# microsoft/SpeechT5

Measured on AMD Instinct MI355X. Metric: audio-sec/s fwd+bwd SpeechT5-Base, higher is better.
Workload: dtype bf16

## Files before the change

### include/speecht5_hip.h

```cpp
#ifndef SPEECHT5_HIP_H
#define SPEECHT5_HIP_H
#include <stdint.h>
#ifdef __cplusplus
extern "C" {
#endif

#define ST5_F32 0
#define ST5_BF16 1

#define ST5_ACT_NONE 0
#define ST5_ACT_GELU 1
#define ST5_ACT_RELU 2
#define ST5_ACT_TANH 3
#define ST5_ACT_LRELU_01 4
#define ST5_ACT_LRELU_001 5

#define ST5_GEMM_A_KSTRIDED 1
#define ST5_GEMM_B_KSTRIDED 2
#define ST5_GEMM_OUT_F32 4
#define ST5_GEMM_DACT 8
#define ST5_GEMM_DEFERRABLE 16

typedef struct st5_operand {
  const void* ptr;
// ... 124 lines not shown
                               const uint8_t* kpm, int32_t B, int32_t H, int32_t T, int32_t S, int32_t head_dim, int32_t nb,
                               int32_t maxrel, int32_t causal, int32_t lds, float scale, float dropout_p, uint64_t seed,
                               const float* gate, int32_t dkv_live, int dtype, void* stream, void* stream2);

int st5_conv0_gn_gelu_fwd(const float* wav, const float* w, const float* gamma, const float* beta, void* out,
                          float* stats, void* ws, int32_t B, int32_t S, int32_t C, int32_t k, int32_t stride,
                          float eps, int dtype, void* stream);
int st5_conv0_gn_gelu_bwd(const float* wav, const float* w, const float* gamma, const float* beta,
                          const float* stats, const void* dY, float* dw, float* dgamma, float* dbeta, void* ws,
                          int32_t B, int32_t S, int32_t C, int32_t k, int32_t stride, float gscale, int dtype,
                          void* stream);
int32_t st5_conv0_mom_count(int32_t k);
int st5_conv0_gn_gelu_fwd_m(const float* wav, const float* w, const float* gamma, const float* beta, void* out, float* stats, double* mom,
                            void* ws, int32_t B, int32_t S, int32_t C, int32_t k, int32_t stride, float eps, int dtype, void* stream);
int st5_conv0_gn_gelu_bwd_m(const float* wav, const float* w, const float* gamma, const float* beta, const float* stats, const double* mom,
                            const void* dY, float* dw, float* dgamma, float* dbeta, void* ws, int32_t B, int32_t S, int32_t C, int32_t k,
                            int32_t stride, float gscale, int dtype, void* stream);
int st5_conv0_gn_gelu_fwd_rows(const float* wav, const int32_t* lens, const float* w, const float* gamma, const float* beta, void* out,
                               float* stats, void* ws, int32_t B, int32_t S, int32_t C, int32_t k, int32_t stride, float eps, int dtype,
                               void* stream);
int st5_conv0_set_mfma(int on);
int st5_conv0_set_fold(int on);
int st5_conv0_set_gelu_table(int on);
int64_t st5_conv0_ws_bytes(int32_t B, int32_t S, int32_t C, int32_t k, int32_t stride);

int st5_cast_from_f32(const float* src, void* dst, int64_t rows, int64_t cols, int32_t transpose, int dtype,
                      void* stream);
int st5_cast_to_f32(const void* src, float* dst, int64_t n, int dtype, void* stream);
int st5_colsum_ws(const void* x, float* out, void* ws, int64_t rows, int32_t cols, int64_t ld, float scale,
                  int32_t accumulate, int dtype, void* stream);
int st5_colsum_ws_gate(const void* x, float* out, void* ws, int64_t rows, int32_t cols, int64_t ld, float scale, int32_t accumulate,
                       const float* gate, int dtype, void* stream);
int64_t st5_colsum_ws_bytes(int64_t rows, int32_t cols);
int st5_sumsq(const void* x, float* out, int64_t n, float scale, int32_t accumulate, int dtype, void* stream);
int st5_axpby(const void* x, void* y, int64_t n, float a, float b, int dtype, void* stream);
int st5_select(const float* keep_dev, const void* a, const void* b, void* y, int64_t nbytes, void* stream);
int st5_select_bwd(const float* keep_dev, const void* g, void* ga, void* gb, int64_t nbytes, void* stream);
int st5_skip_grad(const float* keep_dev, const void* g, void* dx, int64_t nbytes, void* stream);
int st5_act_fwd(const void* x, void* y, int64_t n, int32_t act, int dtype, void* stream);
int st5_act_bwd(const void* dy, const void* x, void* dx, int64_t n, int32_t act, int dtype, void* stream);
int st5_channel_affine(const void* x, const float* a, const float* b, void* y, int64_t rows, int32_t cols, int32_t act,
                       int dtype, void* stream);
int st5_dropout(const void* x, void* y, int64_t n, float p, uint64_t seed, int dtype, void* stream);
int st5_masked_fill_rows(void* x, const uint8_t* mask, const float* v, int64_t rows, int32_t cols, int dtype,
                         void* stream);
int st5_masked_fill_rows_bwd(void* dx, const uint8_t* mask, float* dv, int64_t rows, int32_t cols, int dtype,
                             void* stream);
int st5_add_table_rows(const void* x, const float* table, const int32_t* idx, void* y, int64_t rows, int32_t cols,
                       float scale, int dtype, void* stream);
int st5_add_table_rows_dev(const void* x, const float* table, const int32_t* idx, void* y, int64_t rows, int32_t cols,
                           const float* scale_dev, int dtype, void* stream);
int st5_embed_rows(const float* table, const int32_t* tok, const float* pos, const int32_t* pidx, void* y,
                   int64_t rows, int32_t cols, float emb_scale, float pos_scale, int dtype, void* stream);
int st5_embed_rows_bwd(const void* dy, const int32_t* tok, float* dtable, int64_t rows, int32_t cols, float scale,
                       int dtype, void* stream);
int st5_embed_rows_bwd_det(const void* dy, const int32_t* tok, float* dtable, int64_t rows, int32_t cols, int32_t vocab, float scale,
                           int dtype, void* stream);
int st5_embed_rows_bwd_det_w(const void* dy, const int32_t* tok, float* dtable, int64_t rows, int32_t cols, int32_t vocab, float scale,
                             const float* row_w, int32_t rw_div, int32_t rw_mod, int dtype, void* stream);
int st5_gather3(const float* src, void* dst, int32_t A, int32_t B, int32_t C, int64_t sa, int64_t sb, int64_t sc, int64_t off,
                int32_t accumulate, int dtype, void* stream);
int st5_zero_time_edges(void* x, int32_t B, int32_t Tp, int32_t C, int32_t head, int32_t tail_start, int dtype, void* stream);
int st5_unfold_rows(const float* wav, void* out, int32_t B, int32_t S, int32_t k, int32_t stride, int32_t kpad, int dtype,
                    void* stream);
int st5_pad_time(const void* src, void* dst, int32_t B, int32_t T, int32_t C, int32_t pad_l, int32_t pad_r,
                 int dtype, void* stream);
// ... 154 lines not shown
```

### speecht5_amd/csrc/flash_attn2.hip

```cpp
#include "common.h"
#include "../../include/speecht5_hip.h"

#ifndef FA2_ABL
#define FA2_ABL 0
#endif
#ifdef FA2_DMA_NOP
#define FA2_AFTER_DMA(p) asm volatile("s_nop 7\n\ts_nop 7" ::"v"(p) : "memory")
#else
#define FA2_AFTER_DMA(p)
#endif
namespace fa2 {

constexpr int HD = 64;
constexpr int KT = 64;
constexpr int TILE_B = KT * HD * 2;
constexpr int QP_PAD = 8;
constexpr int WIN = 104;
constexpr int WCH = 13;
constexpr int SCR_B = 7168;
constexpr float LOG2E = 1.4426950408889634f;
constexpr float LN2 = 0.6931471805599453f;
constexpr unsigned int PAIR_MUL = 0x9E3779B1u;

typedef __attribute__((address_space(3))) void* lds_ptr_t;
// ... 506 lines not shown
  block_coords(xb_, bh);
  const int b = bh / a.H, h = bh % a.H;
  const int qblk = xb_ * 128;
  const int qw0 = qblk + wave * 32;
  const int qi = qw0 + ql;
  const int qc = qi < a.T ? qi : a.T - 1;
  const bool qvalid = qi < a.T;

  bf16x8 qf[4], dof[4];
#pragma unroll
  for (int ks = 0; ks < 4; ++ks) {
    qf[ks] = *reinterpret_cast<const bf16x8*>(a.q + ((long long)b * a.T + qc) * a.q_ld + h * HD + ks * 16 + hi * 8);
    dof[ks] = *reinterpret_cast<const bf16x8*>(a.dout + ((long long)b * a.T + qc) * a.do_ld + h * HD + ks * 16 + hi * 8);
  }
  const float lse2 = a.lse[(long long)bh * a.T + qc] * LOG2E;
  float dsum;
  if (a.dvec_in_dq) {
    float part = 0.f;
#pragma unroll
    for (int ks = 0; ks < 4; ++ks) {
      const bf16x8 of = *reinterpret_cast<const bf16x8*>(a.o + ((long long)b * a.T + qc) * a.o_ld + h * HD + ks * 16 + hi * 8);
#pragma unroll
      for (int e = 0; e < 8; ++e) part = fmaf((float)dof[ks][e], (float)of[e], part);
    }
    dsum = part + __shfl_xor(part, 32, 64);
    if (qvalid && hi == 0) a.dvec[(long long)bh * a.T + qi] = dsum;
  } else {
    dsum = a.dvec[(long long)bh * a.T + qc];
  }

  if (BIAS && a.dvec_in_dq) {
    const int nrows = a.T - qblk < 128 ? a.T - qblk : 128;
    uint4* zp = reinterpret_cast<uint4*>(a.dqp + ((long long)bh * a.T + qblk) * a.nb);
    const int n16 = nrows * (a.nb >> 3);
    for (int i = tid; i < n16; i += 256) zp[i] = make_uint4(0u, 0u, 0u, 0u);
    asm volatile("s_waitcnt vmcnt(0)" ::: "memory");
    __builtin_amdgcn_s_barrier();
  }
  int nkeys = a.S;
  if (a.causal) {
    const int qmax = (qblk + 127 < a.T ? qblk + 127 : a.T - 1) + (a.S - a.T);
    nkeys = qmax + 1 < a.S ? qmax + 1 : a.S;
  }
  const int ntiles = (nkeys + KT - 1) / KT;
  const bf16_t* kbase = a.k + (long long)b * a.S * a.k_ld + h * HD;
  const bf16_t* vbase = a.v + (long long)b * a.S * a.v_ld + h * HD;
  TileStager ts;
  ts.init(wave, lane);
  const int nbp = a.nb + 2 * QP_PAD;
  const bf16_t* qpb = BIAS ? a.qp + (long long)bh * a.T * nbp : nullptr;
  WinStager wsg;
  if (BIAS) wsg.init(lane, qw0, a.T, nbp);
  float blo = 0.f, bhi = 0.f;
  if (BIAS) {
    blo = (float)qpb[(long long)qc * nbp];
    bhi = (float)qpb[(long long)qc * nbp + QP_PAD + a.nb];
  }
  TrAddr tra;
  tra.init(lane);
  int koff[2][2];
#pragma unroll
  for (int dt = 0; dt < 2; ++dt) {
    koff[dt][0] = tra.off(4 * hi, dt);
    koff[dt][1] = tra.off(8 + 4 * hi, dt);
  }
  const uint8_t* mrow = a.kpm ? a.kpm + (long long)b * a.S : nullptr;
  unsigned int raw_next = kpm_raw(mrow, lane, a.S);

  ts.issue(kbase, a.k_ld, 0, a.S, kbuf, wave);
  ts.issue(vbase, a.v_ld, 0, a.S, vbuf, wave);
// ... 683 lines not shown
```

### speecht5_amd/csrc/norm.hip

```cpp
#include "common.h"
#include "../../include/speecht5_hip.h"

namespace {

constexpr int MAXCH = 8;

template <typename T, int NCH>
__device__ __forceinline__ void load_row(const T* row, int cols, int lane, bool vec, float (&v)[NCH][8]) {
#pragma unroll
  for (int i = 0; i < NCH; ++i) {
    const int c = i * 512 + lane * 8;
    if (c < cols) {
      if (vec) load8f<T>(row + c, v[i]);
      else {
#pragma unroll
        for (int e = 0; e < 8; ++e) v[i][e] = (c + e < cols) ? Elem<T>::to_f(row[c + e]) : 0.f;
      }
    } else {
#pragma unroll
      for (int e = 0; e < 8; ++e) v[i][e] = 0.f;
    }
  }
}
template <typename T, int NCH>
// ... 467 lines not shown
        }
        const float mu = mean[r], rs = rstd[r];
#pragma unroll
        for (int e = 0; e < 8; ++e) acc[e] += b[e] * (a[e] - mu) * rs;
      } else {
#pragma unroll
        for (int e = 0; e < 8; ++e) acc[e] += a[e];
      }
    }
  }
#pragma unroll
  for (int e = 0; e < 8; ++e) red[ty][tx * 8 + e] = acc[e];
  __syncthreads();
  const int c = threadIdx.x;
  if (blockIdx.x * 256 + c < cols) {
    float s = 0.f;
#pragma unroll
    for (int j = 0; j < 8; ++j) s += red[j][c];
    part[(long long)blockIdx.y * cols + blockIdx.x * 256 + c] = s;
  }
}
__global__ void colreduce_final_kernel(const float* __restrict__ part, float* __restrict__ out, int nsplit, int cols,
                                       float scale, int accumulate, const float* __restrict__ gate = nullptr) {
  const int c = blockIdx.x * blockDim.x + threadIdx.x;
  if (c >= cols) return;
  if (st5_gate_dropped(gate)) {
    if (!accumulate) out[c] = 0.f;
    return;
  }
  float s = 0.f;
  for (int j = 0; j < nsplit; ++j) s += part[(long long)j * cols + c];
  s *= scale;
  out[c] = accumulate ? out[c] + s : s;
}

int nsplit_for(long long rows) {
  long long n = (rows + 63) / 64;
  if (n < 1) n = 1;
  if (n > 64) n = 64;
  return (int)n;
}

template <typename T, int MODE>
int colreduce(const void* x, const void* dy, const float* mean, const float* rstd, float* out, float* ws,
              long long rows, int cols, long long ld, float scale, int accumulate, hipStream_t s, const float* gate = nullptr) {
  const int ns = nsplit_for(rows);
  dim3 grid((cols + 255) / 256, ns);
  hipLaunchKernelGGL((colreduce_kernel<T, MODE>), grid, dim3(256), 0, s, (const T*)x, (const T*)dy, mean, rstd, ws,
                     rows, cols, ld, gate);
  hipLaunchKernelGGL(colreduce_final_kernel, dim3((cols + 255) / 256), dim3(256), 0, s, ws, out, ns, cols, scale,
                     accumulate, gate);
  HIP_CHECK_LAUNCH();
  return ST5_OK;
}

}

static int layernorm_fwd(const void* x, const float* gamma, const float* beta, void* y, float* mean,
                         float* rstd, int64_t rows, int32_t cols, float eps, int dtype, void* stream, const float* keep, const void* skip,
                         const float* gate = nullptr) {
  if (!x || !y || !gamma || !beta || rows < 0 || cols <= 0 || cols > MAXCH * 512) return ST5_ERR_ARG;
  if (keep && (!skip || cols % 4 != 0 || cols > 2048)) return ST5_ERR_ARG;
  if (gate && ((skip && !keep) || cols % 4 != 0 || cols > 2048)) return ST5_ERR_ARG;
  if (rows == 0) return ST5_OK;
  hipStream_t s = (hipStream_t)stream;
  dim3 grid((unsigned)((rows + 3) / 4));
// ... 226 lines not shown
#undef g_ln_arena_bytes
#undef g_ln_arena_used
extern "C" int st5_layernorm_defer(int enabled, void* stream) {
  (void)stream;
  if (!enabled && g_ln_defer) {
    for (int i = 0; i < g_nlnstates; ++i) { const int rc = ln_flush_state(&g_lnstates[i]); if (rc) return rc; }
  }
  g_ln_defer = enabled != 0;
  return ST5_OK;
}
extern "C" int st5_layernorm_flush(void* stream) { return ln_flush(reinterpret_cast<hipStream_t>(stream)); }
extern "C" int st5_layernorm_set_max_blocks(int n) { if (n < 1 || n > 4096) return ST5_ERR_ARG; g_ln_max_blocks = n; return ST5_OK; }

extern "C" int st5_colsum_ws(const void* x, float* out, void* ws, int64_t rows, int32_t cols, int64_t ld, float scale,
                             int32_t accumulate, int dtype, void* stream) {
  if (!x || !out || !ws || rows < 0 || cols <= 0) return ST5_ERR_ARG;
  hipStream_t s = (hipStream_t)stream;
  if (dtype == ST5_BF16)
    return colreduce<bf16_t, 0>(x, nullptr, nullptr, nullptr, out, (float*)ws, rows, cols, ld, scale, accumulate, s);
  if (dtype == ST5_F32)
    return colreduce<float, 0>(x, nullptr, nullptr, nullptr, out, (float*)ws, rows, cols, ld, scale, accumulate, s);
  return ST5_ERR_ARG;
}
extern "C" int st5_colsum_ws_gate(const void* x, float* out, void* ws, int64_t rows, int32_t cols, int64_t ld, float scale,
                                  int32_t accumulate, const float* gate, int dtype, void* stream) {
  if (!x || !out || !ws || rows < 0 || cols <= 0) return ST5_ERR_ARG;
  hipStream_t s = (hipStream_t)stream;
  if (dtype == ST5_BF16)
    return colreduce<bf16_t, 0>(x, nullptr, nullptr, nullptr, out, (float*)ws, rows, cols, ld, scale, accumulate, s, gate);
  if (dtype == ST5_F32)
    return colreduce<float, 0>(x, nullptr, nullptr, nullptr, out, (float*)ws, rows, cols, ld, scale, accumulate, s, gate);
  return ST5_ERR_ARG;
}
extern "C" int64_t st5_colsum_ws_bytes(int64_t rows, int32_t cols) {
  return (int64_t)nsplit_for(rows) * cols * sizeof(float);
}
```

### speecht5_amd/functional.py

```python
import math
from types import SimpleNamespace

import os
import threading

import torch

from . import hip
from .hip import ACT_GELU, ACT_NONE, ACT_RELU, ACT_TANH

_S = SimpleNamespace(dtype=torch.float32, seed=0x5EED, counter=0, grad_hook=None, boundary_hook=None, side=None, side_raw=0,
                     side_keep=[], side_gens=[], side_n=0, attn_side=None, attn_side_raw=None, slots=None, force_static=False)


def set_compute_dtype(dtype):
    assert dtype in (torch.float32, torch.bfloat16)
    _S.dtype = dtype


def compute_dtype():
    return _S.dtype


def manual_seed(seed):
# ... 1520 lines not shown
    hip.gemm(hip.operand(dS, lds, **zP), hip.operand(kt, kld, off=koff, zs0=S * kld, zs1=hd),
             hip.operand(dqt, dqld, off=dqoff, zs0=T * dqld, zs1=hd), T, hd, S, _dt(dtype), batch=BH, zdiv=H,
             flags=hip.B_KSTRIDED, alpha=alpha)
    if pe is not None:
        hip.gemm(hip.operand(dqp, nb, zs0=H * T * nb, zs1=T * nb), hip.operand(pe, hd),
                 hip.operand(dqt, dqld, off=dqoff, zs0=T * dqld, zs1=hd), T, hd, nb, _dt(dtype), batch=BH, zdiv=H,
                 flags=hip.B_KSTRIDED, alpha=alpha, beta=1.0)
    hip.gemm(hip.operand(dS, lds, **zP), hip.operand(qt, qld, off=qoff, zs0=T * qld, zs1=hd),
             hip.operand(dkt, dkld, off=dkoff, zs0=S * dkld, zs1=hd), S, hd, T, _dt(dtype), batch=BH, zdiv=H,
             flags=hip.A_KSTRIDED | hip.B_KSTRIDED, alpha=alpha)
    if pe is not None and want_dpe:
        part = torch.empty(BH, nb, hd, dtype=torch.float32, device=dev)
        hip.gemm(hip.operand(dqp, nb, zs0=H * T * nb, zs1=T * nb),
                 hip.operand(qt, qld, off=qoff, zs0=T * qld, zs1=hd),
                 hip.operand(part, hd, zs0=H * nb * hd, zs1=nb * hd), nb, hd, T, _dt(dtype), batch=BH, zdiv=H,
                 flags=hip.A_KSTRIDED | hip.B_KSTRIDED | hip.OUT_F32, alpha=alpha)
        g = torch.zeros(nb, hd, dtype=torch.float32, device=dev)
        L = hip.lib()
        ws = hip.workspace(L.st5_colsum_ws_bytes(BH, nb * hd), dev)
        hip.check(L.st5_colsum_ws(part.data_ptr(), g.data_ptr(), ws.data_ptr(), BH, nb * hd, nb * hd, 1.0, 1, hip.F32,
                                  hip.stream()), "st5_colsum_ws")
        return g
    return None



_FLASH = SimpleNamespace(enabled=True)


def set_flash_attention(enabled):
    _FLASH.enabled = bool(enabled)


def _can_flash(dtype, hd, want_probs):
    return _FLASH.enabled and dtype == torch.bfloat16 and hd == 64 and not want_probs


def _eptr(t3):
    t, _ld, off = t3
    return t.data_ptr() + off * t.element_size()


_LOG2E = 1.4426950408889634


def _flash_fwd(q, k, v, B, H, T, S, hd, pe, maxrel, kpm, causal, p_drop, seed, save_qp=False):
    dev = q[0].device
    d = H * hd
    ctx = _gout(torch.empty(B * T, d, dtype=torch.bfloat16, device=dev))
    lse = _gout(torch.empty(B * H, T, dtype=torch.float32, device=dev))
    nb = pe.shape[0] if pe is not None else 0
    qp = _gout(torch.empty(B * H, T, hip.lib().st5_flash_attn_qp_row(nb), dtype=torch.bfloat16, device=dev)) if pe is not None else None
    if hip.gate():
        hip.check(hip.lib().st5_flash_attn_fwd_qp_gate(_eptr(q), q[1], _eptr(k), k[1], _eptr(v), v[1], ctx.data_ptr(), d, lse.data_ptr(),
                                                       hip.ptr(pe), hip.ptr(kpm), B, H, T, S, hd, nb, maxrel, 1 if causal else 0, _ceil8(S),
                                                       hd ** -0.5, p_drop, seed, hip.ptr(qp), hip.gate(), hip.BF16, hip.stream()),
                  "st5_flash_attn_fwd_qp_gate")
        return ctx, lse, (qp if save_qp else None)
    hip.check(hip.lib().st5_flash_attn_fwd_qp(_eptr(q), q[1], _eptr(k), k[1], _eptr(v), v[1], ctx.data_ptr(), d, lse.data_ptr(),
                                              hip.ptr(pe), hip.ptr(kpm), B, H, T, S, hd, nb, maxrel, 1 if causal else 0, _ceil8(S),
                                              hd ** -0.5, p_drop, seed, hip.ptr(qp), hip.BF16, hip.stream()), "st5_flash_attn_fwd_qp")
    return ctx, lse, (qp if save_qp else None)


def set_attention_stream(stream):
    _S.attn_side = stream
# ... 16 lines not shown
    lg = hip.gate()
    dev = dctx.device
    dtype = torch.bfloat16
    d = H * hd
    BH = B * H
    alpha = hd ** -0.5
    dvec = _gout(torch.empty(BH * T, dtype=torch.float32, device=dev))
    dqp = None
    nb = 0
    qt, qld, qoff = q
    if pe is not None:
        nb = pe.shape[0]
        assert qp is not None or not lg, "a gated layer keeps the forward's relative-position table (st5_flash_attn_qp_table carries no gate)"
        if qp is None:
            qp = torch.empty(BH, T, hip.lib().st5_flash_attn_qp_row(nb), dtype=dtype, device=dev)
            hip.check(hip.lib().st5_flash_attn_qp_table(_eptr(q), q[1], pe.data_ptr(), qp.data_ptr(), B, H, T, nb, alpha, hip.BF16,
                                                        hip.stream()), "st5_flash_attn_qp_table")
        dqp = _gout(torch.empty(BH, T, nb, dtype=dtype, device=dev))
    if lg:
        hip.check(hip.lib().st5_flash_attn_bwd_2s_gate(_eptr(q), q[1], _eptr(k), k[1], _eptr(v), v[1], ctx.data_ptr(), d, dctx.data_ptr(), d,
                                                       _eptr(dq), dq[1], _eptr(dk), dk[1], _eptr(dv), dv[1], lse.data_ptr(), dvec.data_ptr(),
                                                       hip.ptr(pe), hip.ptr(qp), hip.ptr(dqp), hip.ptr(kpm), B, H, T, S, hd, nb, maxrel,
                                                       1 if causal else 0, _ceil8(S), alpha, p_drop, seed, lg, 1 if dkv_live else 0, hip.BF16,
                                                       hip.stream(), _attn_side_raw()), "st5_flash_attn_bwd_2s_gate")
    else:
        hip.check(hip.lib().st5_flash_attn_bwd_2s(_eptr(q), q[1], _eptr(k), k[1], _eptr(v), v[1], ctx.data_ptr(), d, dctx.data_ptr(), d,
                                                  _eptr(dq), dq[1], _eptr(dk), dk[1], _eptr(dv), dv[1], lse.data_ptr(), dvec.data_ptr(),
                                                  hip.ptr(pe), hip.ptr(qp), hip.ptr(dqp), hip.ptr(kpm), B, H, T, S, hd, nb, maxrel,
                                                  1 if causal else 0, _ceil8(S), alpha, p_drop, seed, hip.BF16, hip.stream(),
                                                  _attn_side_raw()), "st5_flash_attn_bwd_2s")
    if pe is None:
        return None
    dqt, dqld, dqoff = dq
    if pe_t is not None:
        hip.gemm(hip.operand(dqp, nb, zs0=H * T * nb, zs1=T * nb), hip.operand(pe_t, nb),
                 hip.operand(dqt, dqld, off=dqoff, zs0=T * dqld, zs1=hd), T, hd, nb, hip.BF16, batch=BH, zdiv=H, alpha=alpha, beta=1.0)
    else:
        hip.gemm(hip.operand(dqp, nb, zs0=H * T * nb, zs1=T * nb), hip.operand(pe, hd),
                 hip.operand(dqt, dqld, off=dqoff, zs0=T * dqld, zs1=hd), T, hd, nb, hip.BF16, batch=BH, zdiv=H,
                 flags=hip.B_KSTRIDED, alpha=alpha, beta=1.0)
    if not want_dpe:
        return None
    part = _gout(torch.empty(BH, nb, hd, dtype=torch.float32, device=dev))
    hip.gemm(hip.operand(dqp, nb, zs0=H * T * nb, zs1=T * nb), hip.operand(qt, qld, off=qoff, zs0=T * qld, zs1=hd),
             hip.operand(part, hd, zs0=H * nb * hd, zs1=nb * hd), nb, hd, T, hip.BF16, batch=BH, zdiv=H,
             flags=hip.A_KSTRIDED | hip.B_KSTRIDED | hip.OUT_F32, alpha=alpha)
    g = _gout(torch.empty(nb, hd, dtype=torch.float32, device=dev))
    L = hip.lib()
    ws = hip.workspace(L.st5_colsum_ws_bytes(BH, nb * hd), dev)
    if lg:
        hip.check(L.st5_colsum_ws_gate(part.data_ptr(), g.data_ptr(), ws.data_ptr(), BH, nb * hd, nb * hd, 1.0, 0, lg, hip.F32, hip.stream()),
                  "st5_colsum_ws_gate")
        return g
    hip.check(L.st5_colsum_ws(part.data_ptr(), g.data_ptr(), ws.data_ptr(), BH, nb * hd, nb * hd, 1.0, 0, hip.F32, hip.stream()),
              "st5_colsum_ws")
    return g


class SelfAttentionFunction(torch.autograd.Function):

    @staticmethod
    @_lg_fwd
    def forward(ctx_, qkv, pe, kpm, cfg):
        B, H, T, hd, maxrel, causal, p_drop = cfg[:7]
        d = H * hd
        seed = next_seed() if p_drop > 0 else 0
        assert _LG.keep is None or _can_flash(qkv.dtype, hd, False), "gated layer without the fused attention kernels"
        if _can_flash(qkv.dtype, hd, False):
            ctx, lse, qp = _flash_fwd((qkv, 3 * d, 0), (qkv, 3 * d, d), (qkv, 3 * d, 2 * d), B, H, T, T, hd, pe, maxrel, kpm, causal,
                                      p_drop, seed, save_qp=any(ctx_.needs_input_grad))
            ctx_.save_for_backward(qkv, ctx, lse, pe, kpm, qp)
            ctx_.meta = (cfg, seed, True)
            return ctx
        ctx, probs, pdrop = _attn_fwd((qkv, 3 * d, 0), (qkv, 3 * d, d), (qkv, 3 * d, 2 * d), B, H, T, T, hd, pe, maxrel,
                                      kpm, causal, p_drop, seed)
        ctx_.save_for_backward(qkv, probs, pdrop, pe)
        ctx_.meta = (cfg, seed, False)
        return ctx

    @staticmethod
    @_lg_bwd
    def backward(ctx_, dctx):
        cfg, seed, flash = ctx_.meta
        B, H, T, hd, maxrel, causal, p_drop = cfg[:7]
        pe_t = cfg[7] if len(cfg) > 7 else None
        d = H * hd
        if flash:
            qkv, ctx, lse, pe, kpm, qp = ctx_.saved_tensors
            dqkv = _gout(torch.empty_like(qkv))
            dpe = _flash_bwd(dctx.contiguous(), ctx, lse, (qkv, 3 * d, 0), (qkv, 3 * d, d), (qkv, 3 * d, 2 * d), (dqkv, 3 * d, 0),
                             (dqkv, 3 * d, d), (dqkv, 3 * d, 2 * d), B, H, T, T, hd, pe, pe is not None and ctx_.needs_input_grad[1],
                             maxrel, kpm, causal, p_drop, seed, qp=qp, pe_t=pe_t)
            if dpe is not None and pe.dtype != torch.float32:
                dpe = to_compute(dpe)
            return dqkv, dpe, None, None
        qkv, probs, pdrop, pe = ctx_.saved_tensors
        dqkv = torch.empty_like(qkv)
        dpe = _attn_bwd(dctx.contiguous(), (qkv, 3 * d, 0), (qkv, 3 * d, d), (qkv, 3 * d, 2 * d), (dqkv, 3 * d, 0),
                        (dqkv, 3 * d, d), (dqkv, 3 * d, 2 * d), probs, pdrop, None, B, H, T, T, hd, pe,
                        pe is not None and ctx_.needs_input_grad[1], maxrel, p_drop, seed)
        if dpe is not None and pe.dtype != torch.float32:
            dpe = to_compute(dpe)
        return dqkv, dpe, None, None


class KVShare:

    def __init__(self, n_layers, width, may_skip_layers):
        self.n_layers, self.width, self.may_skip = n_layers, width, may_skip_layers
        self.first = None
        self.grad = None

    def grad_buffer(self, like):
        if self.grad is None:
            self.grad = (torch.zeros_like if self.may_skip else torch.empty_like)(like)
        return self.grad


class CrossAttentionFunction(torch.autograd.Function):

    @staticmethod
    @_lg_fwd
    def forward(ctx_, q, kv, kpm, cfg):
        B, H, T, S, hd, p_drop, want_probs = cfg[:7]
        d = H * hd
        kld, koff, share = cfg[7:10] if len(cfg) > 7 else (2 * d, 0, None)
# ... 1398 lines not shown
```

### speecht5_amd/hip.py

```python
import ctypes
import os
from ctypes import POINTER, Structure, byref, c_char_p, c_float, c_int, c_int32, c_int64, c_uint64, c_void_p

import torch

F32, BF16 = 0, 1
ACT_NONE, ACT_GELU, ACT_RELU, ACT_TANH, ACT_LRELU_01, ACT_LRELU_001 = 0, 1, 2, 3, 4, 5
A_KSTRIDED, B_KSTRIDED, OUT_F32, DACT = 1, 2, 4, 8
DEFERRABLE = 16

_LIB_PATH = os.environ.get("ST5_HIP_LIB") or os.path.join(os.path.dirname(os.path.abspath(__file__)), "libspeecht5_hip.so")


class HipLibraryMissing(RuntimeError):
    pass


class HipKernelError(RuntimeError):
    pass


class Operand(Structure):
    _fields_ = [("ptr", c_void_p), ("ld", c_int64), ("rpb", c_int32), ("seg", c_int32),
                ("bstride", c_int64), ("seg_stride", c_int64), ("zs0", c_int64), ("zs1", c_int64)]
# ... 74 lines not shown
    "st5_multi_quant_mxfp8": (c_int, [c_void_p, c_int32, c_int32, c_void_p]),
    "st5_gemm_mxfp8_q": (c_int, [POINTER(GemmParams), c_void_p, c_int64, c_void_p, c_int64, c_void_p, c_int64, c_void_p, c_int64, c_void_p]),
    "st5_layernorm_bwd_add": (c_int, [c_void_p, c_void_p, c_void_p, c_void_p, c_void_p, c_void_p, c_void_p, c_void_p, c_void_p, c_int64, c_int32,
                                      c_void_p, c_int, c_void_p]),
    "st5_layernorm_gelu_fwd": (c_int, [c_void_p, c_void_p, c_void_p, c_void_p, c_void_p, c_void_p, c_int64, c_int32, c_float, c_int, c_void_p]),
    "st5_layernorm_gelu_bwd": (c_int, [c_void_p, c_void_p, c_void_p, c_void_p, c_void_p, c_void_p, c_void_p, c_void_p, c_void_p, c_void_p,
                                       c_int64, c_int32, c_int, c_void_p]),
    "st5_layernorm_fwd_q8": (c_int, [c_void_p, c_void_p, c_void_p, c_void_p, c_void_p, c_void_p, c_void_p, c_void_p, c_int64, c_int32, c_float,
                                     c_void_p]),
    "st5_flash_attn_qp_row": (c_int32, [c_int32]),
    "st5_flash_attn_qp_table": (c_int, [c_void_p, c_int64, c_void_p, c_void_p, c_int32, c_int32, c_int32, c_int32, c_float, c_int, c_void_p]),
    "st5_conv0_gn_gelu_fwd": (c_int, [c_void_p, c_void_p, c_void_p, c_void_p, c_void_p, c_void_p, c_void_p, c_int32,
                                      c_int32, c_int32, c_int32, c_int32, c_float, c_int, c_void_p]),
    "st5_conv0_gn_gelu_bwd": (c_int, [c_void_p, c_void_p, c_void_p, c_void_p, c_void_p, c_void_p, c_void_p, c_void_p,
                                      c_void_p, c_void_p, c_int32, c_int32, c_int32, c_int32, c_int32, c_float, c_int,
                                      c_void_p]),
    "st5_conv0_gn_gelu_fwd_m": (c_int, [c_void_p, c_void_p, c_void_p, c_void_p, c_void_p, c_void_p, c_void_p, c_void_p, c_int32,
                                        c_int32, c_int32, c_int32, c_int32, c_float, c_int, c_void_p]),
    "st5_conv0_gn_gelu_bwd_m": (c_int, [c_void_p, c_void_p, c_void_p, c_void_p, c_void_p, c_void_p, c_void_p, c_void_p, c_void_p,
                                        c_void_p, c_void_p, c_int32, c_int32, c_int32, c_int32, c_int32, c_float, c_int,
                                        c_void_p]),
    "st5_conv0_gn_gelu_fwd_rows": (c_int, [c_void_p, c_void_p, c_void_p, c_void_p, c_void_p, c_void_p, c_void_p, c_void_p, c_int32,
                                           c_int32, c_int32, c_int32, c_int32, c_float, c_int, c_void_p]),
    "st5_conv0_mom_count": (c_int32, [c_int32]),
    "st5_conv0_ws_bytes": (c_int64, [c_int32, c_int32, c_int32, c_int32, c_int32]),
    "st5_conv0_set_mfma": (c_int, [c_int]),
    "st5_conv0_set_fold": (c_int, [c_int]),
    "st5_conv0_set_gelu_table": (c_int, [c_int]),
    "st5_cast_from_f32": (c_int, [c_void_p, c_void_p, c_int64, c_int64, c_int32, c_int, c_void_p]),
    "st5_cast_to_f32": (c_int, [c_void_p, c_void_p, c_int64, c_int, c_void_p]),
    "st5_colsum_ws": (c_int, [c_void_p, c_void_p, c_void_p, c_int64, c_int32, c_int64, c_float, c_int32, c_int,
                              c_void_p]),
    "st5_colsum_ws_bytes": (c_int64, [c_int64, c_int32]),
    "st5_sumsq": (c_int, [c_void_p, c_void_p, c_int64, c_float, c_int32, c_int, c_void_p]),
    "st5_axpby": (c_int, [c_void_p, c_void_p, c_int64, c_float, c_float, c_int, c_void_p]),
    "st5_select": (c_int, [c_void_p, c_void_p, c_void_p, c_void_p, c_int64, c_void_p]),
    "st5_select_bwd": (c_int, [c_void_p, c_void_p, c_void_p, c_void_p, c_int64, c_void_p]),
    "st5_skip_grad": (c_int, [c_void_p, c_void_p, c_void_p, c_int64, c_void_p]),
    "st5_act_fwd": (c_int, [c_void_p, c_void_p, c_int64, c_int32, c_int, c_void_p]),
    "st5_act_bwd": (c_int, [c_void_p, c_void_p, c_void_p, c_int64, c_int32, c_int, c_void_p]),
    "st5_channel_affine": (c_int, [c_void_p, c_void_p, c_void_p, c_void_p, c_int64, c_int32, c_int32, c_int, c_void_p]),
    "st5_dropout": (c_int, [c_void_p, c_void_p, c_int64, c_float, c_uint64, c_int, c_void_p]),
    "st5_masked_fill_rows": (c_int, [c_void_p, c_void_p, c_void_p, c_int64, c_int32, c_int, c_void_p]),
    "st5_masked_fill_rows_bwd": (c_int, [c_void_p, c_void_p, c_void_p, c_int64, c_int32, c_int, c_void_p]),
    "st5_add_table_rows": (c_int, [c_void_p, c_void_p, c_void_p, c_void_p, c_int64, c_int32, c_float, c_int,
                                   c_void_p]),
    "st5_add_table_rows_dev": (c_int, [c_void_p, c_void_p, c_void_p, c_void_p, c_int64, c_int32, c_void_p, c_int, c_void_p]),
    "st5_embed_rows": (c_int, [c_void_p, c_void_p, c_void_p, c_void_p, c_void_p, c_int64, c_int32, c_float, c_float,
                               c_int, c_void_p]),
    "st5_embed_rows_bwd": (c_int, [c_void_p, c_void_p, c_void_p, c_int64, c_int32, c_float, c_int, c_void_p]),
    "st5_embed_rows_bwd_det": (c_int, [c_void_p, c_void_p, c_void_p, c_int64, c_int32, c_int32, c_float, c_int, c_void_p]),
    "st5_unfold_rows": (c_int, [c_void_p, c_void_p, c_int32, c_int32, c_int32, c_int32, c_int32, c_int, c_void_p]),
    "st5_pad_time": (c_int, [c_void_p, c_void_p, c_int32, c_int32, c_int32, c_int32, c_int32, c_int, c_void_p]),
    "st5_pad_time_act": (c_int, [c_void_p, c_void_p, c_int32, c_int32, c_int32, c_int32, c_int32, c_int32, c_int, c_void_p]),
    "st5_zero_halo": (c_int, [c_void_p, c_int32, c_int32, c_int32, c_int32, c_int32, c_int, c_void_p]),
    "st5_ragged_pad_act": (c_int, [c_void_p, c_void_p, c_void_p, c_int64, c_int32, c_int32, c_int32, c_int32, c_int32, c_int, c_void_p]),
    "st5_ragged_zero_gaps": (c_int, [c_void_p, c_void_p, c_void_p, c_int64, c_int64, c_int32, c_int32, c_int, c_void_p]),
    "st5_ragged_gather_rows": (c_int, [c_void_p, c_void_p, c_void_p, c_int64, c_int64, c_int32, c_int32, c_int, c_void_p]),
    "st5_conv1d_narrow": (c_int, [c_void_p, c_int64, c_int32, c_void_p, c_void_p, c_void_p, c_int64, c_int32, c_void_p, c_int64, c_int32,
                                  c_int32, c_int32, c_int32, c_int32, c_int32, c_int32, c_float, c_float, c_int32, c_void_p]),
    "st5_conv1d_cout1": (c_int, [c_void_p, c_int64, c_int32, c_void_p, c_void_p, c_void_p, c_int32, c_int32, c_int32, c_int32, c_int32,
                                 c_float, c_int32, c_void_p]),
    "st5_ragged_rows": (c_int, [c_void_p, c_void_p, c_void_p, c_void_p, c_int32, c_int32, c_int32, c_int32, c_int32, c_int32, c_uint64, c_void_p]),
    "st5_tail_mask": (c_int, [c_void_p, c_void_p, c_int32, c_int32, c_int32, c_void_p]),
    "st5_stft_frames": (c_int, [c_void_p, c_void_p, c_int32, c_int32, c_int32, c_int32, c_void_p]),
    "st5_stft_magnitude": (c_int, [c_void_p, c_void_p, c_int64, c_int32, c_int32, c_void_p]),
# ... 334 lines not shown
```

Measured before the change: 2939.

## Fuse relative-position attention backward into one MFMA kernel and skip dead dqp zeroing

```diff
diff --git a/include/speecht5_hip.h b/include/speecht5_hip.h
--- a/include/speecht5_hip.h
+++ b/include/speecht5_hip.h
@@ -180,6 +180,11 @@
 int st5_colsum_ws_gate(const void* x, float* out, void* ws, int64_t rows, int32_t cols, int64_t ld, float scale, int32_t accumulate,
                        const float* gate, int dtype, void* stream);
 int64_t st5_colsum_ws_bytes(int64_t rows, int32_t cols);
+int st5_colsum_ws_bf16(const void* x, void* out, void* ws, int64_t rows, int32_t cols, int64_t ld, float scale, const float* gate,
+                       int dtype, void* stream);
+int st5_relpos_bwd_supported(int32_t nb, int32_t head_dim, int dtype);
+int st5_relpos_bwd(const void* dqp, const void* pe_t, const void* q, int64_t q_ld, void* dq, int64_t dq_ld, float* part, int32_t B,
+                   int32_t H, int32_t T, int32_t nb, int32_t head_dim, float alpha, const float* gate, int dtype, void* stream);
 int st5_sumsq(const void* x, float* out, int64_t n, float scale, int32_t accumulate, int dtype, void* stream);
 int st5_axpby(const void* x, void* y, int64_t n, float a, float b, int dtype, void* stream);
 int st5_select(const float* keep_dev, const void* a, const void* b, void* y, int64_t nbytes, void* stream);
diff --git a/speecht5_amd/csrc/flash_attn2.hip b/speecht5_amd/csrc/flash_attn2.hip
--- a/speecht5_amd/csrc/flash_attn2.hip
+++ b/speecht5_amd/csrc/flash_attn2.hip
@@ -562,10 +562,27 @@
   if (BIAS && a.dvec_in_dq) {
     const int nrows = a.T - qblk < 128 ? a.T - qblk : 128;
     uint4* zp = reinterpret_cast<uint4*>(a.dqp + ((long long)bh * a.T + qblk) * a.nb);
-    const int n16 = nrows * (a.nb >> 3);
-    for (int i = tid; i < n16; i += 256) zp[i] = make_uint4(0u, 0u, 0u, 0u);
-    asm volatile("s_waitcnt vmcnt(0)" ::: "memory");
-    __builtin_amdgcn_s_barrier();
+    const int nch = a.nb >> 3;
+    bool stored = true;
+    if (!a.causal && a.T == a.S) {
+      for (int r = wave; r < nrows; r += 4) {
+        const int lo = qblk + r - (a.S - 1) + a.maxrel, hi = qblk + r + a.maxrel;
+        const int cl = lo > 1 ? (lo - 1) >> 3 : -1;
+        const int cu = hi < a.nb - 2 ? (hi + 1) >> 3 : nch;
+        if (cl < 0 && cu >= nch) continue;
+        uint4* zr = zp + r * nch;
+        for (int c = lane; c < nch; c += 64)
+          if (c <= cl || c >= cu) zr[c] = make_uint4(0u, 0u, 0u, 0u);
+      }
+      stored = qblk + nrows - 1 - (a.S - 1) + a.maxrel > 1 || qblk + a.maxrel < a.nb - 2;
+    } else {
+      const int n16 = nrows * nch;
+      for (int i = tid; i < n16; i += 256) zp[i] = make_uint4(0u, 0u, 0u, 0u);
+    }
+    if (stored) {
+      asm volatile("s_waitcnt vmcnt(0)" ::: "memory");
+      __builtin_amdgcn_s_barrier();
+    }
   }
   int nkeys = a.S;
   if (a.causal) {
diff --git a/speecht5_amd/csrc/norm.hip b/speecht5_amd/csrc/norm.hip
--- a/speecht5_amd/csrc/norm.hip
+++ b/speecht5_amd/csrc/norm.hip
@@ -523,6 +523,17 @@
   for (int j = 0; j < nsplit; ++j) s += part[(long long)j * cols + c];
   s *= scale;
   out[c] = accumulate ? out[c] + s : s;
+}
+
+__global__ void colreduce_final_bf16_kernel(const float* __restrict__ part, bf16_t* __restrict__ out, int nsplit, int cols, float scale,
+                                            const float* __restrict__ gate = nullptr) {
+  const int c = blockIdx.x * blockDim.x + threadIdx.x;
+  if (c >= cols) return;
+  if (st5_gate_dropped(gate)) { out[c] = (bf16_t)0.f; return; }
+  float s = 0.f;
+  for (int j = 0; j < nsplit; ++j) s += part[(long long)j * cols + c];
+  s *= scale;
+  out[c] = (bf16_t)s;
 }
 
 int nsplit_for(long long rows) {
@@ -815,6 +826,25 @@
     return colreduce<float, 0>(x, nullptr, nullptr, nullptr, out, (float*)ws, rows, cols, ld, scale, accumulate, s, gate);
   return ST5_ERR_ARG;
 }
+extern "C" int st5_colsum_ws_bf16(const void* x, void* out, void* ws, int64_t rows, int32_t cols, int64_t ld, float scale,
+                                  const float* gate, int dtype, void* stream) {
+  if (!x || !out || !ws || rows < 0 || cols <= 0) return ST5_ERR_ARG;
+  hipStream_t s = (hipStream_t)stream;
+  const int ns = nsplit_for(rows);
+  dim3 grid((cols + 255) / 256, ns);
+  if (dtype == ST5_BF16)
+    hipLaunchKernelGGL((colreduce_kernel<bf16_t, 0>), grid, dim3(256), 0, s, (const bf16_t*)x, (const bf16_t*)nullptr, nullptr, nullptr,
+                       (float*)ws, rows, cols, ld, gate);
+  else if (dtype == ST5_F32)
+    hipLaunchKernelGGL((colreduce_kernel<float, 0>), grid, dim3(256), 0, s, (const float*)x, (const float*)nullptr, nullptr, nullptr,
+                       (float*)ws, rows, cols, ld, gate);
+  else
+    return ST5_ERR_ARG;
+  hipLaunchKernelGGL(colreduce_final_bf16_kernel, dim3((cols + 255) / 256), dim3(256), 0, s, (const float*)ws, (bf16_t*)out, ns, cols,
+                     scale, gate);
+  HIP_CHECK_LAUNCH();
+  return ST5_OK;
+}
 extern "C" int64_t st5_colsum_ws_bytes(int64_t rows, int32_t cols) {
   return (int64_t)nsplit_for(rows) * cols * sizeof(float);
 }
diff --git a/speecht5_amd/csrc/relpos_bwd.hip b/speecht5_amd/csrc/relpos_bwd.hip
--- /dev/null
+++ b/speecht5_amd/csrc/relpos_bwd.hip
@@ -0,0 +1,256 @@
+#include "common.h"
+#include "../../include/speecht5_hip.h"
+
+#pragma clang fp contract(off)
+
+namespace {
+
+typedef __attribute__((address_space(3))) void* lds_ptr_t;
+typedef const __attribute__((address_space(1))) void* gbl_ptr_t;
+typedef __attribute__((ext_vector_type(4))) short s16x4;
+
+constexpr int RP_HD = 64;
+constexpr int RP_ROWS = 64;
+constexpr int RP_MAXNB = 320;
+constexpr int RP_QTILE_B = RP_ROWS * RP_HD * 2;
+constexpr int RP_MAXG = RP_MAXNB / 8 / 4;
+constexpr int RP_NTW = 5;
+
+__device__ __attribute__((aligned(256))) char rp_zero_page[256];
+
+__device__ __forceinline__ bf16x8 rp_read128(const unsigned addr) {
+  bf16x8 v;
+  asm volatile("ds_read_b128 %0, %1" : "=v"(v) : "v"(addr) : "memory");
+  return v;
+}
+__device__ __forceinline__ s16x4 rp_read_tr(const unsigned addr) {
+  s16x4 v;
+  asm volatile("ds_read_b64_tr_b16 %0, %1" : "=v"(v) : "v"(addr) : "memory");
+  return v;
+}
+__device__ __forceinline__ bf16x8 rp_join(const s16x4 lo, const s16x4 hi) {
+  union { struct { s16x4 a, b; } s; bf16x8 v; } u;
+  u.s.a = lo; u.s.b = hi;
+  return u.v;
+}
+
+template <bool WANT_PART>
+__global__ __launch_bounds__(256) void relpos_bwd_kernel(const bf16_t* __restrict__ dqp, const bf16_t* __restrict__ pe_t,
+                                                         const bf16_t* __restrict__ q, const long long q_ld, bf16_t* __restrict__ dq,
+                                                         const long long dq_ld, float* __restrict__ part, const int H, const int T,
+                                                         const int nb, const float alpha, const float* __restrict__ gate) {
+  if (st5_gate_dropped(gate)) return;
+  extern __shared__ __attribute__((aligned(16))) char smem[];
+  const int tid = threadIdx.x, lane = tid & 63;
+  const int wave = __builtin_amdgcn_readfirstlane(tid >> 6);
+  const int bh = blockIdx.x, b = bh / H, h = bh - b * H;
+  const int rowb = nb * 2;
+  const int tile_b = RP_ROWS * rowb;
+  const int cpr = nb >> 3;
+  const bool swz = (nb & 63) == 0;
+  auto fz = [&](int row) { return swz ? ((row >> 1) & 7) : 0; };
+  auto fq = [](int row) { return ((row >> 1) & 1) * 4; };
+  char* const dbuf = smem;
+  char* const qbuf = smem + 2 * tile_b;
+  char* const pbuf = qbuf + 2 * RP_QTILE_B;
+  const unsigned lds0 = (unsigned)(size_t)(lds_ptr_t)smem;
+  const unsigned d_lds = lds0, q_lds = lds0 + 2 * tile_b, p_lds = q_lds + 2 * RP_QTILE_B;
+
+  for (int i = tid; i < RP_HD * cpr; i += 256) {
+    const int r = i / cpr, c = i - r * cpr;
+    const u32x4 v = *reinterpret_cast<const u32x4*>(pe_t + (long long)r * nb + c * 8);
+    *reinterpret_cast<u32x4*>(pbuf + r * rowb + ((c ^ fz(r)) << 4)) = v;
+  }
+
+  const int ngroups = nb >> 3;
+  int pk[RP_MAXG];
+#pragma unroll
+  for (int i = 0; i < RP_MAXG; ++i) {
+    const int pch = (wave + 4 * i) * 64 + lane;
+    const int r = pch / cpr, cp = pch - r * cpr;
+    pk[i] = (r << 20) | (r * nb + ((cp ^ fz(r)) << 3));
+  }
+  const bf16_t* const dqp_bh = dqp + (long long)bh * T * nb;
+  const bf16_t* const q_bh = q + (long long)b * T * q_ld + h * RP_HD;
+  bf16_t* const dq_bh = dq + (long long)b * T * dq_ld + h * RP_HD;
+  const bf16_t* const zero = reinterpret_cast<const bf16_t*>(rp_zero_page);
+  const int qrow_l = lane >> 3, qchunk_l = lane & 7;
+  auto issue = [&](const int t0, const int buf) {
+    const bf16_t* const src0 = dqp_bh + (long long)t0 * nb;
+    char* const dst = dbuf + buf * tile_b;
+#pragma unroll
+    for (int i = 0; i < RP_MAXG; ++i) {
+      const int g = wave + 4 * i;
+      if (g < ngroups) {
+        const int r = pk[i] >> 20;
+        const bf16_t* const src = t0 + r < T ? src0 + (pk[i] & 0xfffff) : zero;
+        __builtin_amdgcn_global_load_lds((gbl_ptr_t)src, (lds_ptr_t)(dst + g * 1024), 16, 0, 0);
+      }
+    }
+    if (WANT_PART) {
+      char* const qdst = qbuf + buf * RP_QTILE_B;
+#pragma unroll
+      for (int i = 0; i < 2; ++i) {
+        const int g = wave + 4 * i;
+        const int r = g * 8 + qrow_l;
+        const bf16_t* const src = t0 + r < T ? q_bh + (long long)(t0 + r) * q_ld + ((qchunk_l ^ fq(r)) << 3) : zero;
+        __builtin_amdgcn_global_load_lds((gbl_ptr_t)src, (lds_ptr_t)(qdst + g * 1024), 16, 0, 0);
+      }
+    }
+  };
+
+  const int l31 = lane & 31, hf = lane >> 5;
+  const int th = wave >> 1, dh = wave & 1;
+  const int drow = dh * 32 + l31, trow = th * 32 + l31;
+  const unsigned pe_row = p_lds + drow * rowb, tq_row = trow * rowb;
+  const int fzp = fz(drow), fzt = fz(trow);
+  const int nks = nb >> 4;
+  const int ntn = (nb + 31) >> 5;
+  int nvalid = ntn - (wave >> 1) * RP_NTW;
+  nvalid = nvalid < 0 ? 0 : (nvalid > RP_NTW ? RP_NTW : nvalid);
+  const int nt0 = (wave >> 1) * RP_NTW, dt = wave & 1;
+  const int tg = (lane >> 4) & 1, tj = (lane & 15) >> 2, tq = lane & 3;
+  const int mloc = 2 * tg + (tq >> 1), sub8 = (tq & 1) * 8;
+  f32x16 pacc[RP_NTW];
+#pragma unroll
+  for (int i = 0; i < RP_NTW; ++i)
+#pragma unroll
+    for (int r = 0; r < 16; ++r) pacc[i][r] = 0.f;
+
+  __syncthreads();
+  const int ntl = (T + RP_ROWS - 1) / RP_ROWS;
+  issue(0, 0);
+  for (int it = 0; it < ntl; ++it) {
+    const int t0 = it * RP_ROWS, cur = it & 1;
+    const int tabs = t0 + trow;
+    const bool tok = tabs < T;
+    bf16_t* const dq_row = dq_bh + (long long)(tok ? tabs : 0) * dq_ld + dh * 32 + 4 * hf;
+    u32x2 old[4];
+#pragma unroll
+    for (int rr = 0; rr < 4; ++rr) { old[rr][0] = 0u; old[rr][1] = 0u; }
+    if (tok) {
+#pragma unroll
+      for (int rr = 0; rr < 4; ++rr) old[rr] = *reinterpret_cast<const u32x2*>(dq_row + 8 * rr);
+    }
+    asm volatile("s_waitcnt vmcnt(0)" ::: "memory");
+    __builtin_amdgcn_s_barrier();
+    asm volatile("" : "+v"(old[0]), "+v"(old[1]), "+v"(old[2]), "+v"(old[3]));
+    if (it + 1 < ntl) issue(t0 + RP_ROWS, cur ^ 1);
+
+    const unsigned dcur = d_lds + cur * tile_b;
+    {
+      f32x16 acc;
+#pragma unroll
+      for (int r = 0; r < 16; ++r) acc[r] = 0.f;
+      const unsigned tb = dcur + tq_row;
+      int ks = 0;
+      for (; ks + 2 <= nks; ks += 2) {
+        const int c0 = 2 * ks + hf, c1 = c0 + 2;
+        bf16x8 a0 = rp_read128(pe_row + ((c0 ^ fzp) << 4)), b0 = rp_read128(tb + ((c0 ^ fzt) << 4));
+        bf16x8 a1 = rp_read128(pe_row + ((c1 ^ fzp) << 4)), b1 = rp_read128(tb + ((c1 ^ fzt) << 4));
+        asm volatile("s_waitcnt lgkmcnt(0)" : "+v"(a0), "+v"(b0), "+v"(a1), "+v"(b1) :: "memory");
+        acc = __builtin_amdgcn_mfma_f32_32x32x16_bf16(a0, b0, acc, 0, 0, 0);
+        acc = __builtin_amdgcn_mfma_f32_32x32x16_bf16(a1, b1, acc, 0, 0, 0);
+      }
+      if (ks < nks) {
+        const int c0 = 2 * ks + hf;
+        bf16x8 a0 = rp_read128(pe_row + ((c0 ^ fzp) << 4)), b0 = rp_read128(tb + ((c0 ^ fzt) << 4));
+        asm volatile("s_waitcnt lgkmcnt(0)" : "+v"(a0), "+v"(b0) :: "memory");
+        acc = __builtin_amdgcn_mfma_f32_32x32x16_bf16(a0, b0, acc, 0, 0, 0);
+      }
+      if (tok) {
+#pragma unroll
+        for (int rr = 0; rr < 4; ++rr) {
+          bf16x4 o;
+#pragma unroll
+          for (int e = 0; e < 4; ++e) {
+            const float ov = bf16_bits_to_f((e & 1) ? (old[rr][e >> 1] >> 16) : (old[rr][e >> 1] & 0xffffu));
+            float x = fmaf(acc[4 * rr + e], alpha, 0.f);
+            x = fmaf(1.f, ov, x);
+            o[e] = (bf16_t)x;
+          }
+          *reinterpret_cast<bf16x4*>(dq_row + 8 * rr) = o;
+        }
+      }
+    }
+    if (WANT_PART) {
+      const unsigned qcur = q_lds + cur * RP_QTILE_B;
+#pragma unroll
+      for (int kk = 0; kk < 4; ++kk) {
+        const int r0 = 16 * kk + 8 * hf + tj, r1 = r0 + 4;
+        const int f0 = fz(r0), f1 = fz(r1);
+        const unsigned qa0 = qcur + r0 * 128 + (((dt * 4 + mloc) ^ fq(r0)) << 4) + sub8;
+        const unsigned qa1 = qcur + r1 * 128 + (((dt * 4 + mloc) ^ fq(r1)) << 4) + sub8;
+        const unsigned da0 = dcur + r0 * rowb + ((mloc ^ (f0 & 3)) << 4) + sub8, x0 = (f0 & 4) << 4;
+        const unsigned da1 = dcur + r1 * rowb + ((mloc ^ (f1 & 3)) << 4) + sub8, x1 = (f1 & 4) << 4;
+        s16x4 blo = rp_read_tr(qa0), bhi = rp_read_tr(qa1);
+        s16x4 alo[RP_NTW], ahi[RP_NTW];
+#pragma unroll
+        for (int i = 0; i < RP_NTW; ++i) {
+          alo[i] = s16x4{0, 0, 0, 0}; ahi[i] = s16x4{0, 0, 0, 0};
+          if (i < nvalid) {
+            const unsigned nto = (unsigned)(nt0 + i) << 6;
+            alo[i] = rp_read_tr(da0 + (nto ^ x0));
+            ahi[i] = rp_read_tr(da1 + (nto ^ x1));
+          }
+        }
+        asm volatile("s_waitcnt lgkmcnt(0)" : "+v"(blo), "+v"(bhi), "+v"(alo[0]), "+v"(ahi[0]), "+v"(alo[1]), "+v"(ahi[1]),
+                     "+v"(alo[2]), "+v"(ahi[2]), "+v"(alo[3]), "+v"(ahi[3]), "+v"(alo[4]), "+v"(ahi[4]) :: "memory");
+        const bf16x8 fb = rp_join(blo, bhi);
+#pragma unroll
+        for (int i = 0; i < RP_NTW; ++i)
+          if (i < nvalid) pacc[i] = __builtin_amdgcn_mfma_f32_32x32x16_bf16(rp_join(alo[i], ahi[i]), fb, pacc[i], 0, 0, 0);
+      }
+    }
+  }
+  if (WANT_PART) {
+    float* const pout = part + (long long)bh * nb * RP_HD + dt * 32 + l31;
+#pragma unroll
+    for (int i = 0; i < RP_NTW; ++i) {
+      if (i < nvalid) {
+#pragma unroll
+        for (int r = 0; r < 16; ++r) {
+          const int n = (nt0 + i) * 32 + (r & 3) + 8 * (r >> 2) + 4 * hf;
+          if (n < nb) pout[(long long)n * RP_HD] = fmaf(pacc[i][r], alpha, 0.f);
+        }
+      }
+    }
+  }
+}
+
+template <bool WANT_PART>
+int launch_relpos_bwd(const void* dqp, const void* pe_t, const void* q, long long q_ld, void* dq, long long dq_ld, float* part, int B,
+                      int H, int T, int nb, float alpha, const float* gate, hipStream_t s) {
+  static bool attr = false;
+  if (!attr) {
+    if (hipFuncSetAttribute((const void*)relpos_bwd_kernel<WANT_PART>, hipFuncAttributeMaxDynamicSharedMemorySize, 160 * 1024) != hipSuccess)
+      return ST5_ERR_LAUNCH;
+    attr = true;
+  }
+  const size_t shm = (size_t)3 * RP_ROWS * nb * 2 + 2 * RP_QTILE_B;
+  hipLaunchKernelGGL(relpos_bwd_kernel<WANT_PART>, dim3(B * H), dim3(256), shm, s, (const bf16_t*)dqp, (const bf16_t*)pe_t,
+                     (const bf16_t*)q, q_ld, (bf16_t*)dq, dq_ld, part, H, T, nb, alpha, gate);
+  HIP_CHECK_LAUNCH();
+  return ST5_OK;
+}
+
+bool rp_aligned(const void* p) { return (reinterpret_cast<uintptr_t>(p) & 15) == 0; }
+
+}
+
+extern "C" int st5_relpos_bwd_supported(int32_t nb, int32_t head_dim, int dtype) {
+  return dtype == ST5_BF16 && head_dim == RP_HD && nb >= 16 && nb <= RP_MAXNB && nb % 16 == 0;
+}
+
+extern "C" int st5_relpos_bwd(const void* dqp, const void* pe_t, const void* q, int64_t q_ld, void* dq, int64_t dq_ld, float* part,
+                              int32_t B, int32_t H, int32_t T, int32_t nb, int32_t head_dim, float alpha, const float* gate, int dtype,
+                              void* stream) {
+  if (!dqp || !pe_t || !q || !dq || B <= 0 || H <= 0 || T <= 0) return ST5_ERR_ARG;
+  if (!st5_relpos_bwd_supported(nb, head_dim, dtype)) return ST5_ERR_ARG;
+  if (!rp_aligned(dqp) || !rp_aligned(pe_t) || !rp_aligned(q) || !rp_aligned(dq) || q_ld % 8 != 0 || dq_ld % 8 != 0 ||
+      (part && !rp_aligned(part)))
+    return ST5_ERR_ALIGN;
+  hipStream_t s = (hipStream_t)stream;
+  if (part) return launch_relpos_bwd<true>(dqp, pe_t, q, q_ld, dq, dq_ld, part, B, H, T, nb, alpha, gate, s);
+  return launch_relpos_bwd<false>(dqp, pe_t, q, q_ld, dq, dq_ld, part, B, H, T, nb, alpha, gate, s);
+}
diff --git a/speecht5_amd/functional.py b/speecht5_amd/functional.py
--- a/speecht5_amd/functional.py
+++ b/speecht5_amd/functional.py
@@ -1576,6 +1576,13 @@
     _FLASH.enabled = bool(enabled)
 
 
+_RELPOS = SimpleNamespace(fused=True)
+
+
+def set_relpos_fused(enabled):
+    _RELPOS.fused = bool(enabled)
+
+
 def _can_flash(dtype, hd, want_probs):
     return _FLASH.enabled and dtype == torch.bfloat16 and hd == 64 and not want_probs
 
@@ -1658,6 +1665,18 @@
     if pe is None:
         return None
     dqt, dqld, dqoff = dq
+    L = hip.lib()
+    if _RELPOS.fused and pe_t is not None and pe.dtype == torch.bfloat16 and L.st5_relpos_bwd_supported(nb, hd, hip.BF16):
+        part = _gout(torch.empty(BH, nb, hd, dtype=torch.float32, device=dev)) if want_dpe else None
+        hip.check(L.st5_relpos_bwd(dqp.data_ptr(), pe_t.data_ptr(), _eptr(q), qld, _eptr(dq), dqld, hip.ptr(part), B, H, T, nb, hd, alpha,
+                                   lg, hip.BF16, hip.stream()), "st5_relpos_bwd")
+        if not want_dpe:
+            return None
+        g = _gout(torch.empty(nb, hd, dtype=torch.bfloat16, device=dev))
+        ws = hip.workspace(L.st5_colsum_ws_bytes(BH, nb * hd), dev)
+        hip.check(L.st5_colsum_ws_bf16(part.data_ptr(), g.data_ptr(), ws.data_ptr(), BH, nb * hd, nb * hd, 1.0, lg, hip.F32, hip.stream()),
+                  "st5_colsum_ws_bf16")
+        return g
     if pe_t is not None:
         hip.gemm(hip.operand(dqp, nb, zs0=H * T * nb, zs1=T * nb), hip.operand(pe_t, nb),
                  hip.operand(dqt, dqld, off=dqoff, zs0=T * dqld, zs1=hd), T, hd, nb, hip.BF16, batch=BH, zdiv=H, alpha=alpha, beta=1.0)
@@ -1672,7 +1691,6 @@
              hip.operand(part, hd, zs0=H * nb * hd, zs1=nb * hd), nb, hd, T, hip.BF16, batch=BH, zdiv=H,
              flags=hip.A_KSTRIDED | hip.B_KSTRIDED | hip.OUT_F32, alpha=alpha)
     g = _gout(torch.empty(nb, hd, dtype=torch.float32, device=dev))
-    L = hip.lib()
     ws = hip.workspace(L.st5_colsum_ws_bytes(BH, nb * hd), dev)
     if lg:
         hip.check(L.st5_colsum_ws_gate(part.data_ptr(), g.data_ptr(), ws.data_ptr(), BH, nb * hd, nb * hd, 1.0, 0, lg, hip.F32, hip.stream()),
@@ -1717,7 +1735,7 @@
             dpe = _flash_bwd(dctx.contiguous(), ctx, lse, (qkv, 3 * d, 0), (qkv, 3 * d, d), (qkv, 3 * d, 2 * d), (dqkv, 3 * d, 0),
                              (dqkv, 3 * d, d), (dqkv, 3 * d, 2 * d), B, H, T, T, hd, pe, pe is not None and ctx_.needs_input_grad[1],
                              maxrel, kpm, causal, p_drop, seed, qp=qp, pe_t=pe_t)
-            if dpe is not None and pe.dtype != torch.float32:
+            if dpe is not None and dpe.dtype != pe.dtype:
                 dpe = to_compute(dpe)
             return dqkv, dpe, None, None
         qkv, probs, pdrop, pe = ctx_.saved_tensors
diff --git a/speecht5_amd/hip.py b/speecht5_amd/hip.py
--- a/speecht5_amd/hip.py
+++ b/speecht5_amd/hip.py
@@ -130,6 +130,10 @@
     "st5_colsum_ws": (c_int, [c_void_p, c_void_p, c_void_p, c_int64, c_int32, c_int64, c_float, c_int32, c_int,
                               c_void_p]),
     "st5_colsum_ws_bytes": (c_int64, [c_int64, c_int32]),
+    "st5_colsum_ws_bf16": (c_int, [c_void_p, c_void_p, c_void_p, c_int64, c_int32, c_int64, c_float, c_void_p, c_int, c_void_p]),
+    "st5_relpos_bwd_supported": (c_int, [c_int32, c_int32, c_int]),
+    "st5_relpos_bwd": (c_int, [c_void_p, c_void_p, c_void_p, c_int64, c_void_p, c_int64, c_void_p, c_int32, c_int32, c_int32, c_int32,
+                       c_int32, c_float, c_void_p, c_int, c_void_p]),
     "st5_sumsq": (c_int, [c_void_p, c_void_p, c_int64, c_float, c_int32, c_int, c_void_p]),
     "st5_axpby": (c_int, [c_void_p, c_void_p, c_int64, c_float, c_float, c_int, c_void_p]),
     "st5_select": (c_int, [c_void_p, c_void_p, c_void_p, c_void_p, c_int64, c_void_p]),
```

New measurement: 2966, median of 6. No clear change (+0.9%).
